# eikehmueller/mlmcpathintegral

Measured on AMD Instinct MI355X. Metric: lattice-site-updates/sec, higher is better.
Workload: dtype f64

## Files before the change

### mlmcpathintegral_amd/csrc/schwinger_perm.hpp

```cpp
#pragma once
#include "lattice_sweep.hpp"

namespace mlmcpi {

#ifdef MLMCPI_STAMPS
__device__ unsigned long long g_stamps[16 * 65536];
#define MLMCPI_STAMP(k)                                                                                            \
  do {                                                                                                             \
    if (threadIdx.x == 0 && blockIdx.y * gridDim.x + blockIdx.x < 65536)                                           \
      g_stamps[(blockIdx.y * gridDim.x + blockIdx.x) * 16 + (k)] = __builtin_amdgcn_s_memrealtime();               \
  } while (0)
#define MLMCPI_STAMP_WHERE()                                                                                       \
  do {                                                                                                             \
    if (threadIdx.x == 0 && blockIdx.y * gridDim.x + blockIdx.x < 65536)                                           \
      g_stamps[(blockIdx.y * gridDim.x + blockIdx.x) * 16 + 15] =                                                  \
          ((unsigned long long)__builtin_amdgcn_s_getreg((20 ) | (0 << 6) | (31 << 11)) << 32) |         \
          __builtin_amdgcn_s_getreg((4 ) | (0 << 6) | (31 << 11));                                        \
  } while (0)
#else
#define MLMCPI_STAMP(k) do { } while (0)
#define MLMCPI_STAMP_WHERE() do { } while (0)
#endif

#ifndef MLMCPI_PERM_U
#define MLMCPI_PERM_U 0
#endif

template <class PG>
struct PermPlane {
  static constexpr int kRow = PG::kPitch * 8, kStep = kRow + 8;
  static constexpr uint32_t QB = (uint32_t)PG::kQRows * kRow;
  static_assert(kStep == (int)PG::kStep * 8, "the stride of a stream");
  uint32_t K;
  __device__ __forceinline__ explicit PermPlane(uint32_t K_) : K(K_) {}
  __device__ __forceinline__ bool has_col(uint32_t C) const { return (C & 1u) ? C <= PG::col_last(K, 1) : C >= PG::col_first(K, 0) && C <= PG::col_last(K, 0); }
  __device__ __forceinline__ bool has_row(uint32_t R) const { return (R & 1u) ? R <= PG::row_last(K, 1) : R >= PG::row_first(K, 0) && R <= PG::row_last(K, 0); }
  __device__ __forceinline__ uint32_t col(uint32_t C) const { return (C & 1u) ? QB + PG::col_u(K, C) * 8u : PG::col_u(K, C) * 8u; }
  __device__ __forceinline__ uint32_t row(uint32_t R) const { return (R & 1u) ? 2u * QB + PG::row_v(K, R) * (uint32_t)kRow : PG::row_v(K, R) * (uint32_t)kRow; }
};

struct PermBuildPos {
  uint32_t c, r, rend, row_off, gj;
  uint32_t cb;
  const double2 *src;
  uint32_t col;
  bool active, owns;
};
template <int NT, class PP>
__device__ __forceinline__ PermBuildPos perm_build_pos(const PP &P, const double2 *__restrict__ src, uint32_t Mt, uint32_t Mx, uint32_t gi0,
                                                       uint32_t gj0, uint32_t W, uint32_t rows) {
  PermBuildPos q;
  const uint32_t wave = __builtin_amdgcn_readfirstlane(threadIdx.x / kWave), lane = threadIdx.x % kWave;
  const uint32_t nwc = W > 63 ? 2 : 1;
  const uint32_t groups = (NT / kWave) >> (nwc - 1);
  const uint32_t g = wave >> (nwc - 1), cw = wave & (nwc - 1);
  static_assert(((NT / kWave) & (NT / kWave - 1)) == 0, "waves per workgroup: a power of two (shifts for divisions)");
  const uint32_t rpg = groups == 4 ? (rows + 3) >> 2 : groups == 8 ? (rows + 7) >> 3 : (rows + groups - 1) / groups;
  q.c = 63 * cw + lane;
  q.r = __builtin_amdgcn_readfirstlane(g * rpg);
  q.rend = __builtin_amdgcn_readfirstlane(g < groups ? min(rows, q.r + rpg) : 0);
  q.active = q.r < q.rend;
  q.owns = lane < 63 && q.c < W && P.has_col(q.c);
  q.cb = P.col(q.c);
  q.src = src;
  q.col = wrap_add(gi0, min(q.c, W), Mt);
  q.gj = __builtin_amdgcn_readfirstlane(wrap_add(gj0, q.r, Mx));
  q.row_off = q.gj * Mt;
  return q;
}
template <int U>
__device__ __forceinline__ void perm_rows_load(PermBuildPos &q, uint32_t Mt, uint32_t Mx, bool first, double2 &cur, double2 (&nxt)[U]) {
  if (!q.active) return;
  if (first) cur = (q.src + q.row_off)[q.col];
#pragma unroll
  for (int u = 0; u < U; ++u) {
    q.gj = q.gj + 1 == Mx ? 0 : q.gj + 1;
    q.row_off = q.gj == 0 ? 0 : q.row_off + Mt;
    if (q.r + u < q.rend) nxt[u] = (q.src + q.row_off)[q.col];
  }
}
template <int U, class PP>
__device__ __forceinline__ void perm_rows_store(PermBuildPos &q, const PP &P, double *plane, double2 &cur, const double2 (&nxt)[U]) {
  if (!q.active) return;
  char *const pb = reinterpret_cast<char *>(plane) + q.cb;
#pragma unroll
  for (int u = 0; u < U; ++u)
    if (q.r + u < q.rend) {
      const double right = wave_rotate_down(cur.y);
      if (q.owns && P.has_row(q.r + u)) *reinterpret_cast<double *>(pb + P.row(q.r + u)) = ((cur.x + right) - nxt[u].x) - cur.y;
      cur = nxt[u];
    }
  q.r += U;
}
template <int NT, int U, bool ONCE, class PP>
__device__ __forceinline__ void perm_build_rows(const PP &P, double *plane, const double2 *__restrict__ src, uint32_t Mt, uint32_t Mx,
                                                uint32_t gi0, uint32_t gj0, uint32_t W, uint32_t rows) {
  PermBuildPos q = perm_build_pos<NT>(P, src, Mt, Mx, gi0, gj0, W, rows);
  double2 cur = make_double2(0., 0.);
  if (ONCE) {
    double2 nxt[U];
    perm_rows_load<U>(q, Mt, Mx, true, cur, nxt);
    perm_rows_store<U>(q, P, plane, cur, nxt);
    return;
  }
  bool first = true;
  while (__builtin_amdgcn_readfirstlane(q.r) < __builtin_amdgcn_readfirstlane(q.rend)) {
    double2 nxt[U];
    perm_rows_load<U>(q, Mt, Mx, first, cur, nxt);
    perm_rows_store<U>(q, P, plane, cur, nxt);
    first = false;
  }
}

template <int NT, int RING, int TH = 64>
struct PermTasks {
  using PG = PermGeom<NT, RING, TH>;
  static constexpr int OW = PG::OW, HR = PG::HR, H2 = HR / 2, NW = NT / kWave, NS = (HR + NW - 1) / NW;
  static constexpr int XC = OW - 64;
  static constexpr int L0 = XC * H2, L1 = (XC / 2) * HR;
  static constexpr int NL0 = (L0 + 63) / 64, NL1 = (L1 + 63) / 64;
  static constexpr int WF = HR - NW * (NS - 1);
  static_assert(PG::NV == NS, "slots per thread");
  static_assert(NL0 + NL1 <= NW - WF, "the left-over wave-tasks fit the free last slots");
  uint32_t wave, lane, c_mu0, c_mu1, r_lo;
  __device__ PermTasks() {
    wave = __builtin_amdgcn_readfirstlane(threadIdx.x / kWave);
    lane = threadIdx.x % kWave;
    c_mu0 = lane < 32 ? 2 * lane : 2 * (lane - 32) + 1;
    c_mu1 = 2 * (lane & 31u);
    r_lo = lane >> 5;
  }
  __device__ __forceinline__ bool task(int k, bool &mu1, uint32_t &r, uint32_t &c) const {
    const uint32_t m = wave + (uint32_t)(NW * k);
    mu1 = false; r = 0; c = 0;
    if (NW * k + NW - 1 < H2 || m < (uint32_t)H2) {
      r = 2 * m;
      c = c_mu0;
      return true;
    }
    if (m < (uint32_t)HR) {
      mu1 = true;
      r = 2 * (m - H2) + r_lo;
      c = c_mu1;
      return true;
    }
    if (XC > 0 && k == NS - 1) {
      const uint32_t j = wave - (uint32_t)WF;
      if (j < (uint32_t)NL0) {
        const uint32_t L = 64 * j + lane;
        r = 2 * (L / (XC ? XC : 1));
        c = 64 + L % (XC ? XC : 1);
        return L < (uint32_t)L0;
      }
      if (j < (uint32_t)(NL0 + NL1)) {
        const uint32_t L = 64 * (j - NL0) + lane;
        mu1 = true;
        r = L / (XC > 1 ? XC / 2 : 1);
        c = 64 + 2 * (L % (XC > 1 ? XC / 2 : 1));
        return L < (uint32_t)L1;
      }
    }
    return false;
  }
  __device__ __forceinline__ bool valid(int k) const {
    bool mu1; uint32_t r, c;
    return task(k, mu1, r, c);
  }
  __device__ __forceinline__ bool is_mu1(int k) const {
    bool mu1; uint32_t r, c;
    task(k, mu1, r, c);
    return mu1;
  }
  __device__ __forceinline__ void coords(int k, uint32_t &r, uint32_t &c) const {
    bool mu1;
    task(k, mu1, r, c);
  }
};

template <int STEP>
__device__ __forceinline__ void perm_gather5(uint32_t pa, uint32_t px, uint32_t px2, double &S, double &X, double &X2) {
  double a0 = lds_read_f64<0>(pa), x0 = lds_read_f64<0>(px), y0 = lds_read_f64<0>(px2);
  double a1 = lds_read_f64<STEP>(pa), x1 = lds_read_f64<STEP>(px), y1 = lds_read_f64<STEP>(px2);
  double a2 = lds_read_f64<2 * STEP>(pa), x2 = lds_read_f64<2 * STEP>(px), y2 = lds_read_f64<2 * STEP>(px2);
  double a3 = lds_read_f64<3 * STEP>(pa), x3 = lds_read_f64<3 * STEP>(px), y3 = lds_read_f64<3 * STEP>(px2);
  double a4 = lds_read_f64<4 * STEP>(pa), x4 = lds_read_f64<4 * STEP>(px), y4 = lds_read_f64<4 * STEP>(px2);
  asm volatile("s_waitcnt lgkmcnt(0)"
               : "+v"(a0), "+v"(x0), "+v"(y0), "+v"(a1), "+v"(x1), "+v"(y1), "+v"(a2), "+v"(x2), "+v"(y2), "+v"(a3), "+v"(x3), "+v"(y3),
                 "+v"(a4), "+v"(x4), "+v"(y4)
               :
               : "memory");
  S += a0; X += x0; X2 += y0;
  S += a1; X += x1; X2 += y1;
  S += a2; X += x2; X2 += y2;
  S += a3; X += x3; X2 += y3;
  S += a4; X += x4; X2 += y4;
}
__device__ __forceinline__ void perm_gather1(uint32_t pa, uint32_t px, uint32_t px2, double &S, double &X, double &X2) {
  double a0 = lds_read_f64<0>(pa), x0 = lds_read_f64<0>(px), y0 = lds_read_f64<0>(px2);
  asm volatile("s_waitcnt lgkmcnt(0)" : "+v"(a0), "+v"(x0), "+v"(y0) : : "memory");
  S += a0; X += x0; X2 += y0;
}

template <int NT, int RING, int TH = 64>
__device__ __forceinline__ void perm_sweeps(double *plane, const double2 *__restrict__ src, uint32_t Mt, uint32_t Mx, uint32_t i0,
                                            uint32_t j0, uint32_t K, double2 (&res)[2][PermGeom<NT, RING, TH>::NV]) {
  using PG = PermGeom<NT, RING, TH>;
  using PP = PermPlane<PG>;
  constexpr int HR = PG::HR, NV = PG::NV;
  constexpr int kGroups = NT / kWave / 2;
  constexpr int U = MLMCPI_PERM_U ? MLMCPI_PERM_U : (2 * HR + 4 * (int)kPermMaxK + kGroups - 1) / kGroups;
  const uint32_t W = PG::width(K), rows = PG::rows(K), H = RING + 2 * K;
  const PP P(K);
  auto back = [](uint32_t x, uint32_t h, uint32_t n) { return h <= n ? (x >= h ? x - h : x + n - h) : (x + n - h % n) % n; };
  const uint32_t gi0 = back(i0, H, Mt), gj0 = back(j0, H, Mx);
  const uint32_t oi0 = back(i0, RING, Mt), oj0 = back(j0, RING, Mx);
  const PermTasks<NT, RING, TH> tasks;
  const char *const src_b = reinterpret_cast<const char *>(src);
  const bool small_lattice = Mx < (uint32_t)(2 * HR + 2) || Mt < (uint32_t)(PG::OW + 2);
  auto load_theta_of = [&](int h, double2 (&th)[NV], auto small) {
#pragma unroll
    for (int k = 0; k < NV; ++k) {
      if (!tasks.valid(k)) continue;
      uint32_t r, c;
      tasks.coords(k, r, c);
      uint32_t gr = oj0 + r + h * HR, gc = oi0 + c;
      gr = min(gr, gr - Mx);
      gc = min(gc, gc - Mt);
      if ((bool)small) {
        gr = min(gr, gr - Mx); gr = min(gr, gr - Mx);
        gc = min(gc, gc - Mt); gc = min(gc, gc - Mt);
      }
      const uint32_t o = (gr * Mt + gc) * 16u;
      if (!tasks.is_mu1(k)) {
        const uint32_t o2 = gr + 1 == Mx ? o - gr * Mt * 16u : o + Mt * 16u;
        th[k] = make_double2(*reinterpret_cast<const double *>(src_b + o), *reinterpret_cast<const double *>(src_b + o2));
      } else {
        const uint32_t o2 = gc + 1 == Mt ? o - gc * 16u : o + 16u;
        th[k] = make_double2(*reinterpret_cast<const double *>(src_b + o + 8u), *reinterpret_cast<const double *>(src_b + o2 + 8u));
      }
    }
  };
  auto load_theta = [&](int h, double2 (&th)[NV]) {
    if (small_lattice) load_theta_of(h, th, std::true_type{}); else load_theta_of(h, th, std::false_type{});
  };
  auto gather = [&](int h, double2 (&d)[NV]) {
    const uint32_t lds0 = (uint32_t)(uintptr_t)plane;
#pragma unroll
    for (int k = 0; k < NV; ++k) {
      if (!tasks.valid(k)) continue;
      uint32_t r, c;
      tasks.coords(k, r, c);
      const uint32_t ro = r + (uint32_t)(h * HR), cq = c >> 1, rq = ro >> 1;
      uint32_t a, x, x2;
      if (!tasks.is_mu1(k)) {
        const uint32_t cb = (c & 1u) ? PP::QB + ((uint32_t)(PG::OW / 2 - 1) - cq) * 8u : cq * 8u;
        x = cb + rq * (uint32_t)PP::kRow;
        x2 = x + (uint32_t)PP::kRow;
        a = cb + 2u * PP::QB + ((uint32_t)(HR - 1) - rq) * (uint32_t)PP::kRow;
      } else {
        const uint32_t rb = (ro & 1u) ? 2u * PP::QB + ((uint32_t)(HR - 1) - rq) * (uint32_t)PP::kRow : (rq + 1u) * (uint32_t)PP::kRow;
        x = rb + cq * 8u;
        x2 = x + 8u;
        a = rb + PP::QB + ((uint32_t)(PG::OW / 2) - cq) * 8u;
      }
      uint32_t pa = lds0 + a, px = lds0 + x, px2 = lds0 + x2;
      double S = 0.0, X = 0.0, X2 = 0.0;
      uint32_t s = 0;
      for (; s + 5 <= K; s += 5) {
        perm_gather5<PP::kStep>(pa, px, px2, S, X, X2);
        pa += 5 * PP::kStep;
        px += 5 * PP::kStep;
        px2 += 5 * PP::kStep;
      }
      for (; s < K; ++s) {
        perm_gather1(pa, px, px2, S, X, X2);
        pa += PP::kStep;
        px += PP::kStep;
        px2 += PP::kStep;
      }
      d[k] = tasks.is_mu1(k) ? make_double2(X - S, X2 - S) : make_double2(S - X, S - X2);
    }
  };
  auto finish = [&](const double2 (&th)[NV], double2 (&d)[NV]) {
#pragma unroll
    for (int k = 0; k < NV; ++k)
      if (tasks.valid(k)) d[k] = make_double2(mod_2pi_fast(th[k].x + d[k].x), mod_2pi_fast(th[k].y + d[k].y));
  };

  perm_build_rows<NT, U, MLMCPI_PERM_U == 0>(P, plane, src, Mt, Mx, gi0, gj0, W, rows);
  double2 th[NV];
  load_theta(0, th);
  __syncthreads();
  MLMCPI_STAMP(1);
  gather(0, res[0]);
  finish(th, res[0]);
  MLMCPI_STAMP(2);
  load_theta(1, th);
  gather(1, res[1]);
  finish(th, res[1]);
}

template <int NT, int RING, int TH = 64>
__device__ __forceinline__ void perm_store_image(double *th0, double *th1, const double2 (&res)[2][PermGeom<NT, RING, TH>::NV]) {
  using PG = PermGeom<NT, RING, TH>;
  constexpr int OW = PG::OW, HR = PG::HR, NV = PG::NV;
  const PermTasks<NT, RING, TH> tasks;
#pragma unroll
  for (int h = 0; h < 2; ++h)
#pragma unroll
    for (int k = 0; k < NV; ++k) {
      if (!tasks.valid(k)) continue;
      uint32_t r, c;
      tasks.coords(k, r, c);
      const uint32_t o = (r + h * HR) * OW + c;
      if (!tasks.is_mu1(k)) {
        th0[o] = res[h][k].x;
        th0[o + OW] = res[h][k].y;
      } else {
        th1[o] = res[h][k].x;
        th1[o + 1] = res[h][k].y;
      }
    }
}

}
```

Before: 1107 billion.

## Reassign mu0 row tasks contiguously per wave to reuse adjacent-row gather sums

Remaps the mu0 row tasks so each wave owns a contiguous block of R0 row-pairs instead of strided rows. The gather loop then walks those rows in reverse, so each row's second-row sum (X2) equals the first-row sum X already computed for the row above. That drops one of the three LDS read streams for most mu0 tasks, cutting LDS read traffic in the gather phase. The cost is a changed task-to-wave mapping, which may alter LDS bank access patterns, plus extra control logic and register pressure.

```diff
diff --git a/mlmcpathintegral_amd/csrc/schwinger_perm.hpp b/mlmcpathintegral_amd/csrc/schwinger_perm.hpp
--- a/mlmcpathintegral_amd/csrc/schwinger_perm.hpp
+++ b/mlmcpathintegral_amd/csrc/schwinger_perm.hpp
@@ -116,6 +116,7 @@
 struct PermTasks {
   using PG = PermGeom<NT, RING, TH>;
   static constexpr int OW = PG::OW, HR = PG::HR, H2 = HR / 2, NW = NT / kWave, NS = (HR + NW - 1) / NW;
+  static constexpr int R0 = H2 / NW;
   static constexpr int XC = OW - 64;
   static constexpr int L0 = XC * H2, L1 = (XC / 2) * HR;
   static constexpr int NL0 = (L0 + 63) / 64, NL1 = (L1 + 63) / 64;
@@ -133,8 +134,8 @@
   __device__ __forceinline__ bool task(int k, bool &mu1, uint32_t &r, uint32_t &c) const {
     const uint32_t m = wave + (uint32_t)(NW * k);
     mu1 = false; r = 0; c = 0;
-    if (NW * k + NW - 1 < H2 || m < (uint32_t)H2) {
-      r = 2 * m;
+    if (k < R0 || m < (uint32_t)H2) {
+      r = 2 * (k < R0 ? wave * (uint32_t)R0 + (uint32_t)k : m);
       c = c_mu0;
       return true;
     }
@@ -171,6 +172,7 @@
     task(k, mu1, r, c);
     return mu1;
   }
+  static constexpr bool inherits(int k) { return k + 1 < R0; }
   __device__ __forceinline__ void coords(int k, uint32_t &r, uint32_t &c) const {
     bool mu1;
     task(k, mu1, r, c);
@@ -200,6 +202,28 @@
   asm volatile("s_waitcnt lgkmcnt(0)" : "+v"(a0), "+v"(x0), "+v"(y0) : : "memory");
   S += a0; X += x0; X2 += y0;
 }
+template <int STEP>
+__device__ __forceinline__ void perm_gather5(uint32_t pa, uint32_t px, double &S, double &X) {
+  double a0 = lds_read_f64<0>(pa), x0 = lds_read_f64<0>(px);
+  double a1 = lds_read_f64<STEP>(pa), x1 = lds_read_f64<STEP>(px);
+  double a2 = lds_read_f64<2 * STEP>(pa), x2 = lds_read_f64<2 * STEP>(px);
+  double a3 = lds_read_f64<3 * STEP>(pa), x3 = lds_read_f64<3 * STEP>(px);
+  double a4 = lds_read_f64<4 * STEP>(pa), x4 = lds_read_f64<4 * STEP>(px);
+  asm volatile("s_waitcnt lgkmcnt(0)"
+               : "+v"(a0), "+v"(x0), "+v"(a1), "+v"(x1), "+v"(a2), "+v"(x2), "+v"(a3), "+v"(x3), "+v"(a4), "+v"(x4)
+               :
+               : "memory");
+  S += a0; X += x0;
+  S += a1; X += x1;
+  S += a2; X += x2;
+  S += a3; X += x3;
+  S += a4; X += x4;
+}
+__device__ __forceinline__ void perm_gather1(uint32_t pa, uint32_t px, double &S, double &X) {
+  double a0 = lds_read_f64<0>(pa), x0 = lds_read_f64<0>(px);
+  asm volatile("s_waitcnt lgkmcnt(0)" : "+v"(a0), "+v"(x0) : : "memory");
+  S += a0; X += x0;
+}
 
 template <int NT, int RING, int TH = 64>
 __device__ __forceinline__ void perm_sweeps(double *plane, const double2 *__restrict__ src, uint32_t Mt, uint32_t Mx, uint32_t i0,
@@ -245,8 +269,11 @@
   };
   auto gather = [&](int h, double2 (&d)[NV]) {
     const uint32_t lds0 = (uint32_t)(uintptr_t)plane;
-#pragma unroll
-    for (int k = 0; k < NV; ++k) {
+    using T = PermTasks<NT, RING, TH>;
+    double Xup = 0.0;
+#pragma unroll
+    for (int kk = 0; kk < NV; ++kk) {
+      const int k = kk < T::R0 ? T::R0 - 1 - kk : kk;
       if (!tasks.valid(k)) continue;
       uint32_t r, c;
       tasks.coords(k, r, c);
@@ -266,18 +293,33 @@
       uint32_t pa = lds0 + a, px = lds0 + x, px2 = lds0 + x2;
       double S = 0.0, X = 0.0, X2 = 0.0;
       uint32_t s = 0;
-      for (; s + 5 <= K; s += 5) {
-        perm_gather5<PP::kStep>(pa, px, px2, S, X, X2);
-        pa += 5 * PP::kStep;
-        px += 5 * PP::kStep;
-        px2 += 5 * PP::kStep;
-      }
-      for (; s < K; ++s) {
-        perm_gather1(pa, px, px2, S, X, X2);
-        pa += PP::kStep;
-        px += PP::kStep;
-        px2 += PP::kStep;
-      }
+      if (T::inherits(k)) {
+        for (; s + 5 <= K; s += 5) {
+          perm_gather5<PP::kStep>(pa, px, S, X);
+          pa += 5 * PP::kStep;
+          px += 5 * PP::kStep;
+        }
+        for (; s < K; ++s) {
+          perm_gather1(pa, px, S, X);
+          pa += PP::kStep;
+          px += PP::kStep;
+        }
+        X2 = Xup;
+      } else {
+        for (; s + 5 <= K; s += 5) {
+          perm_gather5<PP::kStep>(pa, px, px2, S, X, X2);
+          pa += 5 * PP::kStep;
+          px += 5 * PP::kStep;
+          px2 += 5 * PP::kStep;
+        }
+        for (; s < K; ++s) {
+          perm_gather1(pa, px, px2, S, X, X2);
+          pa += PP::kStep;
+          px += PP::kStep;
+          px2 += PP::kStep;
+        }
+      }
+      Xup = X;
       d[k] = tasks.is_mu1(k) ? make_double2(X - S, X2 - S) : make_double2(S - X, S - X2);
     }
   };
```

Result: no change. 1113 billion (median of 6 runs) (+0.6%).
